# leggedrobotics/wild_visual_navigation

Measured on NVIDIA H100. Metric: frames/sec end-to-end (DINO feat + seg + MLP train-step) at 448x448, higher is better.
Workload: dtype bf16 operands / fp32 accumulate (ViT, STEGO head, per-pixel MLP); fp32 (k-means, train step)

## Files before the change

wild_visual_navigation_b200/csrc/attention_wgmma.cu:

```cuda
#include <stdlib.h>

#include "attention.h"
#include "common.cuh"
#include "host_common.h"

namespace wvn {

namespace {

constexpr int kThreads = 384;
constexpr int kConsumerWarps = 8;
constexpr int kTileQ = 128;
constexpr int kTileKV = 128;
constexpr int kDh = 64;
constexpr uint32_t kQBytes = kTileQ * kDh * 2;
constexpr uint32_t kKBytes = kTileKV * kDh * 2;
constexpr uint32_t kVBytes = kDh * kTileKV * 2;
constexpr int kStages = 4;
constexpr uint32_t kOffQ = 0;
constexpr uint32_t kOffK = kOffQ + kQBytes;
constexpr uint32_t kOffV = kOffK + kStages * kKBytes;
constexpr uint32_t kOffBar = kOffV + kStages * kVBytes;
constexpr uint32_t kSmemBytes = kOffBar + 256 + 1024 ;

__device__ __forceinline__ float fast_exp2(float x) {
  float y;
  asm("ex2.approx.ftz.f32 %0, %1;" : "=f"(y) : "f"(x));
  return y;
}

__device__ __forceinline__ float quad_max(float v) {
  v = fmaxf(v, __shfl_xor_sync(0xffffffffu, v, 1));
  return fmaxf(v, __shfl_xor_sync(0xffffffffu, v, 2));
}

template <bool MASKED>
__device__ __forceinline__ void softmax_scores(float (&s)[64], float (&m)[2], float (&l)[2], float (&alpha)[2],
                                               const float sl2, const int valid, const int q) {
  if (MASKED) {
#pragma unroll
    for (int j = 0; j < 16; ++j)
#pragma unroll
      for (int e = 0; e < 2; ++e)
        if (8 * j + 2 * q + e >= valid) s[4 * j + e] = s[4 * j + 2 + e] = -INFINITY;
  }
  float neg_m[2];
#pragma unroll
  for (int h = 0; h < 2; ++h) {
    float mx = s[2 * h];
#pragma unroll
    for (int j = 0; j < 16; ++j) mx = fmaxf(mx, fmaxf(s[4 * j + 2 * h], s[4 * j + 2 * h + 1]));
    mx = fmaxf(quad_max(mx), m[h]);
    alpha[h] = fast_exp2((m[h] - mx) * sl2);
    m[h] = mx;
    neg_m[h] = -mx * sl2;
  }
  float sum[2] = {0.f, 0.f};
#pragma unroll
  for (int j = 0; j < 16; ++j) {
#pragma unroll
    for (int h = 0; h < 2; ++h) {
      const float e0 = fast_exp2(fmaf(s[4 * j + 2 * h], sl2, neg_m[h]));
      const float e1 = fast_exp2(fmaf(s[4 * j + 2 * h + 1], sl2, neg_m[h]));
      sum[h] += e0 + e1;
      s[4 * j + 2 * h] = e0;
      s[4 * j + 2 * h + 1] = e1;
    }
  }
#pragma unroll
  for (int h = 0; h < 2; ++h) l[h] = fmaf(l[h], alpha[h], sum[h]);
}

__device__ __forceinline__ void rescale_o(float (&o)[32], const float (&alpha)[2]) {
#pragma unroll
  for (int j = 0; j < 8; ++j) {
    o[4 * j + 0] *= alpha[0];
    o[4 * j + 1] *= alpha[0];
    o[4 * j + 2] *= alpha[1];
    o[4 * j + 3] *= alpha[1];
  }
}

__device__ __forceinline__ void pack_p(const float (&s)[64], uint32_t (&p)[32]) {
#pragma unroll
  for (int j = 0; j < 16; ++j)
#pragma unroll
    for (int h = 0; h < 2; ++h)
      p[4 * (j >> 1) + 2 * (j & 1) + h] = pack_bf16x2(s[4 * j + 2 * h], s[4 * j + 2 * h + 1]);
}

__global__ void __launch_bounds__(kThreads, 1)
attention_kernel(const __grid_constant__ CUtensorMap tmap_q, const __grid_constant__ CUtensorMap tmap_k,
                 const __grid_constant__ CUtensorMap tmap_v, const AttnArgs args) {
  extern __shared__ uint8_t smem_raw[];
  uint8_t* smem = reinterpret_cast<uint8_t*>((reinterpret_cast<uintptr_t>(smem_raw) + 1023) & ~uintptr_t(1023));
  uint64_t* bars = reinterpret_cast<uint64_t*>(smem + kOffBar);
  uint64_t* q_full = bars;
  uint64_t* kv_full = bars + 1;
  uint64_t* kv_empty = bars + 1 + kStages;

  const int warp = threadIdx.x >> 5, lane = threadIdx.x & 31;
  const int ntiles = args.npad / kTileQ;
  const int q_tile = args.reverse ? ntiles - 1 - static_cast<int>(blockIdx.x) : static_cast<int>(blockIdx.x);
  const int bh = args.reverse ? static_cast<int>(gridDim.y) - 1 - static_cast<int>(blockIdx.y) : static_cast<int>(blockIdx.y);
  const int num_kv = args.npad / kTileKV;

  if (threadIdx.x == 0) {
    tma_prefetch_desc(&tmap_q);
    tma_prefetch_desc(&tmap_k);
    tma_prefetch_desc(&tmap_v);
    mbar_init(q_full, 1);
    for (int i = 0; i < kStages; ++i) {
      mbar_init(&kv_full[i], 1);
      mbar_init(&kv_empty[i], kConsumerWarps);
    }
    fence_mbar_init();
  }
  __syncthreads();

  if (warp < 4) {
    setmaxnreg_dec<40>();
    if (warp == 0) {
      if (elect_one_sync()) {
        mbar_arrive_expect_tx(q_full, kQBytes);
        tma_load_2d(&tmap_q, q_full, smem + kOffQ, 0, bh * args.npad + q_tile * kTileQ);
      }
      __syncwarp();
      int stage = 0;
      uint32_t phase = 0;
      for (int j = 0; j < num_kv; ++j) {
        mbar_wait(&kv_empty[stage], phase ^ 1);
        if (elect_one_sync()) {
          mbar_arrive_expect_tx(&kv_full[stage], kKBytes + kVBytes);
          tma_load_2d(&tmap_k, &kv_full[stage], smem + kOffK + stage * kKBytes, 0, bh * args.npad + j * kTileKV);
          tma_load_2d(&tmap_v, &kv_full[stage], smem + kOffV + stage * kVBytes, j * kTileKV, bh * kDh);
          tma_load_2d(&tmap_v, &kv_full[stage], smem + kOffV + stage * kVBytes + kVBytes / 2, j * kTileKV + 64, bh * kDh);
        }
        __syncwarp();
        if (++stage == kStages) { stage = 0; phase ^= 1; }
      }
    }
  } else {
    setmaxnreg_inc<232>();
    const int cwarp = warp - 4;
    const int wg = cwarp >> 2;
    const int q = lane & 3;
    const float sl2 = args.scale_log2;
    float s[64], o[32];
    uint32_t p[32];
    float m[2] = {-INFINITY, -INFINITY}, l[2] = {0.f, 0.f};

    float alpha[2];

    mbar_wait(q_full, 0);
    const uint64_t desc_q = make_sw128_kmajor_desc(smem_u32(smem + kOffQ + wg * 64 * 128));
    auto issue_qk = [&](int st) {
      const uint64_t desc_k = make_sw128_kmajor_desc(smem_u32(smem + kOffK + st * kKBytes));
#pragma unroll
      for (int k = 0; k < kDh / 16; ++k) wgmma_m64n128k16_ss(s, desc_q + 2 * k, desc_k + 2 * k, k != 0 ? 1u : 0u);
      wgmma_commit();
    };
    auto issue_pv = [&](int st, bool accumulate) {
      const uint32_t v_addr = smem_u32(smem + kOffV + st * kVBytes);
#pragma unroll
      for (int k = 0; k < kTileKV / 16; ++k)
        wgmma_m64n64k16_rs(o, p[4 * k], p[4 * k + 1], p[4 * k + 2], p[4 * k + 3],
                           make_sw128_kmajor_desc(v_addr + (k >> 2) * (kVBytes / 2)) + 2 * (k & 3),
                           (accumulate || k != 0) ? 1u : 0u);
      wgmma_commit();
    };
    auto take_turn = [&]() { named_bar_sync(1 + wg, 256); };
    auto pass_turn = [&](bool last) { if (!(last && wg == 1)) named_bar_arrive(2 - wg, 256); };
    if (wg == 1) named_bar_arrive(1, 256);

    mbar_wait(&kv_full[0], 0);
    take_turn();
    wgmma_fence_regs(s);
    wgmma_fence();
    issue_qk(0);
    pass_turn(false);
    wgmma_wait<0>();
    wgmma_fence_regs(s);
    if (num_kv == 1) softmax_scores<true>(s, m, l, alpha, sl2, args.n_valid, q);
    else softmax_scores<false>(s, m, l, alpha, sl2, kTileKV, q);
    pack_p(s, p);

    int stage = 0;
    uint32_t phase = 0;
    for (int j = 1; j < num_kv; ++j) {
      const int prev_stage = stage;
      if (++stage == kStages) { stage = 0; phase ^= 1; }
      mbar_wait(&kv_full[stage], phase);
      take_turn();
      wgmma_fence_regs(s);
      wgmma_fence_regs(o);
      wgmma_fence();
      issue_qk(stage);
      issue_pv(prev_stage, j > 1);
      pass_turn(false);
      wgmma_wait<1>();
      wgmma_fence_regs(s);
      if (j == num_kv - 1) softmax_scores<true>(s, m, l, alpha, sl2, args.n_valid - j * kTileKV, q);
      else softmax_scores<false>(s, m, l, alpha, sl2, kTileKV, q);
      wgmma_wait<0>();
      wgmma_fence_regs(o);
      wgmma_fence_regs(p);
      if (lane == 0) mbar_arrive(&kv_empty[prev_stage]);
      rescale_o(o, alpha);
      pack_p(s, p);
    }
    take_turn();
    wgmma_fence_regs(o);
    wgmma_fence();
    issue_pv(stage, num_kv > 1);
    pass_turn(true);
    wgmma_wait<0>();
    wgmma_fence_regs(o);

    const int frame = bh / args.heads, head = bh - frame * args.heads;
    const int row0 = q_tile * kTileQ + wg * 64 + (cwarp & 3) * 16 + (lane >> 2);
#pragma unroll
    for (int h = 0; h < 2; ++h) {
      float lt = l[h];
      lt += __shfl_xor_sync(0xffffffffu, lt, 1);
      lt += __shfl_xor_sync(0xffffffffu, lt, 2);
      const float inv = 1.f / lt;
      __nv_bfloat16* dst = reinterpret_cast<__nv_bfloat16*>(args.out) +
                           (static_cast<long long>(frame) * args.npad + row0 + 8 * h) * args.ldo + head * kDh + 2 * q;
#pragma unroll
      for (int jj = 0; jj < 8; ++jj)
        *reinterpret_cast<uint32_t*>(dst + 8 * jj) = pack_bf16x2(o[4 * jj + 2 * h] * inv, o[4 * jj + 2 * h + 1] * inv);
    }
  }
}

}

int attention_bf16(const AttnArgs& a, const void* q, const void* k, const void* vt, cudaStream_t stream) {
  WVN_REQUIRE(a.batch > 0 && a.heads > 0, "attention: empty problem");
  WVN_REQUIRE(a.npad % kTileKV == 0 && a.n_valid > 0 && a.n_valid <= a.npad && a.n_valid > a.npad - kTileKV,
              "attention: npad=%d must be a multiple of 128 and n_valid=%d must lie in the last tile", a.npad,
              a.n_valid);
  const long long bh = static_cast<long long>(a.batch) * a.heads;
  WVN_REQUIRE(bh <= 65535, "attention: batch * heads = %lld exceeds the grid's y extent", bh);
  CUtensorMap tq, tk, tv;
  WVN_PROPAGATE(make_tmap_bf16_2d(&tq, q, kDh, bh * a.npad, kDh * 2, 64, kTileQ));
  WVN_PROPAGATE(make_tmap_bf16_2d(&tk, k, kDh, bh * a.npad, kDh * 2, 64, kTileKV));
  WVN_PROPAGATE(make_tmap_bf16_2d(&tv, vt, a.npad, bh * kDh, static_cast<uint64_t>(a.npad) * 2, 64, kDh));
  static bool attr_set = false;
  if (!attr_set) {
    WVN_CHECK_CUDA(cudaFuncSetAttribute(attention_kernel, cudaFuncAttributeMaxDynamicSharedMemorySize, kSmemBytes));
    attr_set = true;
  }
  dim3 grid(a.npad / kTileQ, static_cast<unsigned>(bh));
  prof_begin(PROF_ATTENTION, stream);
  attention_kernel<<<grid, kThreads, kSmemBytes, stream>>>(tq, tk, tv, a);
  prof_end(PROF_ATTENTION, stream);
  WVN_CHECK_LAUNCH("attention_kernel");
  return WVN_OK;
}

}
```

Before: 974.6.

## Make attention kernel persistent with double-buffered Q and TMA output stores

Converts the attention kernel to a persistent grid sized to the SM count. Each CTA loops over (batch*head, q-tile) units, with a double-buffered Q tile so the next unit's first QK^T overlaps the previous unit's final PV. Output is staged through swizzled shared memory and written with TMA stores instead of direct global stores. This aims to remove launch/tail and prologue/epilogue bubbles per tile, at the cost of more shared memory and more complex barrier phase tracking.

```diff
diff --git a/wild_visual_navigation_b200/csrc/attention_wgmma.cu b/wild_visual_navigation_b200/csrc/attention_wgmma.cu
--- a/wild_visual_navigation_b200/csrc/attention_wgmma.cu
+++ b/wild_visual_navigation_b200/csrc/attention_wgmma.cu
@@ -1,4 +1,7 @@
+#include <stdint.h>
 #include <stdlib.h>
+
+#include <algorithm>
 
 #include "attention.h"
 #include "common.cuh"
@@ -16,11 +19,14 @@
 constexpr uint32_t kQBytes = kTileQ * kDh * 2;
 constexpr uint32_t kKBytes = kTileKV * kDh * 2;
 constexpr uint32_t kVBytes = kDh * kTileKV * 2;
+constexpr uint32_t kOBytes = kTileQ * kDh * 2;
+constexpr int kQBufs = 2;
 constexpr int kStages = 4;
 constexpr uint32_t kOffQ = 0;
-constexpr uint32_t kOffK = kOffQ + kQBytes;
+constexpr uint32_t kOffK = kOffQ + kQBufs * kQBytes;
 constexpr uint32_t kOffV = kOffK + kStages * kKBytes;
-constexpr uint32_t kOffBar = kOffV + kStages * kVBytes;
+constexpr uint32_t kOffO = kOffV + kStages * kVBytes;
+constexpr uint32_t kOffBar = kOffO + kOBytes;
 constexpr uint32_t kSmemBytes = kOffBar + 256 + 1024 ;
 
 __device__ __forceinline__ float fast_exp2(float x) {
@@ -91,25 +97,35 @@
 
 __global__ void __launch_bounds__(kThreads, 1)
 attention_kernel(const __grid_constant__ CUtensorMap tmap_q, const __grid_constant__ CUtensorMap tmap_k,
-                 const __grid_constant__ CUtensorMap tmap_v, const AttnArgs args) {
+                 const __grid_constant__ CUtensorMap tmap_v, const __grid_constant__ CUtensorMap tmap_o,
+                 const AttnArgs args) {
   extern __shared__ uint8_t smem_raw[];
   uint8_t* smem = reinterpret_cast<uint8_t*>((reinterpret_cast<uintptr_t>(smem_raw) + 1023) & ~uintptr_t(1023));
   uint64_t* bars = reinterpret_cast<uint64_t*>(smem + kOffBar);
   uint64_t* q_full = bars;
-  uint64_t* kv_full = bars + 1;
-  uint64_t* kv_empty = bars + 1 + kStages;
+  uint64_t* q_empty = bars + kQBufs;
+  uint64_t* kv_full = bars + 2 * kQBufs;
+  uint64_t* kv_empty = bars + 2 * kQBufs + kStages;
 
   const int warp = threadIdx.x >> 5, lane = threadIdx.x & 31;
   const int ntiles = args.npad / kTileQ;
-  const int q_tile = args.reverse ? ntiles - 1 - static_cast<int>(blockIdx.x) : static_cast<int>(blockIdx.x);
-  const int bh = args.reverse ? static_cast<int>(gridDim.y) - 1 - static_cast<int>(blockIdx.y) : static_cast<int>(blockIdx.y);
   const int num_kv = args.npad / kTileKV;
+  const int units = args.batch * args.heads * ntiles;
+  auto unit_coords = [&](int u, int& bh, int& q_tile) {
+    const int ue = args.reverse ? units - 1 - u : u;
+    bh = ue / ntiles;
+    q_tile = ue - bh * ntiles;
+  };
 
   if (threadIdx.x == 0) {
     tma_prefetch_desc(&tmap_q);
     tma_prefetch_desc(&tmap_k);
     tma_prefetch_desc(&tmap_v);
-    mbar_init(q_full, 1);
+    tma_prefetch_desc(&tmap_o);
+    for (int i = 0; i < kQBufs; ++i) {
+      mbar_init(&q_full[i], 1);
+      mbar_init(&q_empty[i], kConsumerWarps);
+    }
     for (int i = 0; i < kStages; ++i) {
       mbar_init(&kv_full[i], 1);
       mbar_init(&kv_empty[i], kConsumerWarps);
@@ -121,23 +137,31 @@
   if (warp < 4) {
     setmaxnreg_dec<40>();
     if (warp == 0) {
-      if (elect_one_sync()) {
-        mbar_arrive_expect_tx(q_full, kQBytes);
-        tma_load_2d(&tmap_q, q_full, smem + kOffQ, 0, bh * args.npad + q_tile * kTileQ);
-      }
-      __syncwarp();
       int stage = 0;
       uint32_t phase = 0;
-      for (int j = 0; j < num_kv; ++j) {
-        mbar_wait(&kv_empty[stage], phase ^ 1);
+      int it = 0;
+      for (int u = blockIdx.x; u < units; u += gridDim.x, ++it) {
+        int bh, q_tile;
+        unit_coords(u, bh, q_tile);
+        const int qb = it & 1;
+        mbar_wait(&q_empty[qb], ((it >> 1) & 1) ^ 1);
         if (elect_one_sync()) {
-          mbar_arrive_expect_tx(&kv_full[stage], kKBytes + kVBytes);
-          tma_load_2d(&tmap_k, &kv_full[stage], smem + kOffK + stage * kKBytes, 0, bh * args.npad + j * kTileKV);
-          tma_load_2d(&tmap_v, &kv_full[stage], smem + kOffV + stage * kVBytes, j * kTileKV, bh * kDh);
-          tma_load_2d(&tmap_v, &kv_full[stage], smem + kOffV + stage * kVBytes + kVBytes / 2, j * kTileKV + 64, bh * kDh);
+          mbar_arrive_expect_tx(&q_full[qb], kQBytes);
+          tma_load_2d(&tmap_q, &q_full[qb], smem + kOffQ + qb * kQBytes, 0, bh * args.npad + q_tile * kTileQ);
         }
         __syncwarp();
-        if (++stage == kStages) { stage = 0; phase ^= 1; }
+        for (int j = 0; j < num_kv; ++j) {
+          mbar_wait(&kv_empty[stage], phase ^ 1);
+          if (elect_one_sync()) {
+            mbar_arrive_expect_tx(&kv_full[stage], kKBytes + kVBytes);
+            tma_load_2d(&tmap_k, &kv_full[stage], smem + kOffK + stage * kKBytes, 0, bh * args.npad + j * kTileKV);
+            tma_load_2d(&tmap_v, &kv_full[stage], smem + kOffV + stage * kVBytes, j * kTileKV, bh * kDh);
+            tma_load_2d(&tmap_v, &kv_full[stage], smem + kOffV + stage * kVBytes + kVBytes / 2, j * kTileKV + 64,
+                        bh * kDh);
+          }
+          __syncwarp();
+          if (++stage == kStages) { stage = 0; phase ^= 1; }
+        }
       }
     }
   } else {
@@ -145,16 +169,12 @@
     const int cwarp = warp - 4;
     const int wg = cwarp >> 2;
     const int q = lane & 3;
+    const bool leader = (threadIdx.x & 127) == 0;
     const float sl2 = args.scale_log2;
     float s[64], o[32];
     uint32_t p[32];
-    float m[2] = {-INFINITY, -INFINITY}, l[2] = {0.f, 0.f};
-
-    float alpha[2];
-
-    mbar_wait(q_full, 0);
-    const uint64_t desc_q = make_sw128_kmajor_desc(smem_u32(smem + kOffQ + wg * 64 * 128));
-    auto issue_qk = [&](int st) {
+
+    auto issue_qk = [&](uint64_t desc_q, int st) {
       const uint64_t desc_k = make_sw128_kmajor_desc(smem_u32(smem + kOffK + st * kKBytes));
 #pragma unroll
       for (int k = 0; k < kDh / 16; ++k) wgmma_m64n128k16_ss(s, desc_q + 2 * k, desc_k + 2 * k, k != 0 ? 1u : 0u);
@@ -172,65 +192,123 @@
     auto take_turn = [&]() { named_bar_sync(1 + wg, 256); };
     auto pass_turn = [&](bool last) { if (!(last && wg == 1)) named_bar_arrive(2 - wg, 256); };
     if (wg == 1) named_bar_arrive(1, 256);
-
-    mbar_wait(&kv_full[0], 0);
+    auto q_desc = [&](int it) {
+      return make_sw128_kmajor_desc(smem_u32(smem + kOffQ + (it & 1) * kQBytes + wg * 64 * 128));
+    };
+    float m[2], l[2], alpha[2];
+    auto first_softmax = [&]() {
+      m[0] = m[1] = -INFINITY;
+      l[0] = l[1] = 0.f;
+      if (num_kv == 1) softmax_scores<true>(s, m, l, alpha, sl2, args.n_valid, q);
+      else softmax_scores<false>(s, m, l, alpha, sl2, kTileKV, q);
+    };
+
+    int stage = 0;
+    uint32_t phase = 0;
+    int it = 0;
+    int u = blockIdx.x;
+    mbar_wait(&q_full[0], 0);
+    mbar_wait(&kv_full[stage], phase);
     take_turn();
     wgmma_fence_regs(s);
     wgmma_fence();
-    issue_qk(0);
+    issue_qk(q_desc(0), stage);
     pass_turn(false);
     wgmma_wait<0>();
     wgmma_fence_regs(s);
-    if (num_kv == 1) softmax_scores<true>(s, m, l, alpha, sl2, args.n_valid, q);
-    else softmax_scores<false>(s, m, l, alpha, sl2, kTileKV, q);
+    first_softmax();
     pack_p(s, p);
 
-    int stage = 0;
-    uint32_t phase = 0;
-    for (int j = 1; j < num_kv; ++j) {
-      const int prev_stage = stage;
+    for (;;) {
+      const uint64_t desc_q = q_desc(it);
+      for (int j = 1; j < num_kv; ++j) {
+        const int prev_stage = stage;
+        if (++stage == kStages) { stage = 0; phase ^= 1; }
+        mbar_wait(&kv_full[stage], phase);
+        take_turn();
+        wgmma_fence_regs(s);
+        wgmma_fence_regs(o);
+        wgmma_fence();
+        issue_qk(desc_q, stage);
+        issue_pv(prev_stage, j > 1);
+        pass_turn(false);
+        wgmma_wait<1>();
+        wgmma_fence_regs(s);
+        if (j == num_kv - 1) softmax_scores<true>(s, m, l, alpha, sl2, args.n_valid - j * kTileKV, q);
+        else softmax_scores<false>(s, m, l, alpha, sl2, kTileKV, q);
+        wgmma_wait<0>();
+        wgmma_fence_regs(o);
+        wgmma_fence_regs(p);
+        if (lane == 0) mbar_arrive(&kv_empty[prev_stage]);
+        rescale_o(o, alpha);
+        pack_p(s, p);
+      }
+      if (lane == 0) mbar_arrive(&q_empty[it & 1]);
+
+      const int next = u + static_cast<int>(gridDim.x);
+      const bool has_next = next < units;
+      const int last_stage = stage;
       if (++stage == kStages) { stage = 0; phase ^= 1; }
-      mbar_wait(&kv_full[stage], phase);
-      take_turn();
-      wgmma_fence_regs(s);
-      wgmma_fence_regs(o);
-      wgmma_fence();
-      issue_qk(stage);
-      issue_pv(prev_stage, j > 1);
-      pass_turn(false);
-      wgmma_wait<1>();
-      wgmma_fence_regs(s);
-      if (j == num_kv - 1) softmax_scores<true>(s, m, l, alpha, sl2, args.n_valid - j * kTileKV, q);
-      else softmax_scores<false>(s, m, l, alpha, sl2, kTileKV, q);
-      wgmma_wait<0>();
-      wgmma_fence_regs(o);
-      wgmma_fence_regs(p);
-      if (lane == 0) mbar_arrive(&kv_empty[prev_stage]);
-      rescale_o(o, alpha);
-      pack_p(s, p);
-    }
-    take_turn();
-    wgmma_fence_regs(o);
-    wgmma_fence();
-    issue_pv(stage, num_kv > 1);
-    pass_turn(true);
-    wgmma_wait<0>();
-    wgmma_fence_regs(o);
-
-    const int frame = bh / args.heads, head = bh - frame * args.heads;
-    const int row0 = q_tile * kTileQ + wg * 64 + (cwarp & 3) * 16 + (lane >> 2);
-#pragma unroll
-    for (int h = 0; h < 2; ++h) {
-      float lt = l[h];
-      lt += __shfl_xor_sync(0xffffffffu, lt, 1);
-      lt += __shfl_xor_sync(0xffffffffu, lt, 2);
-      const float inv = 1.f / lt;
-      __nv_bfloat16* dst = reinterpret_cast<__nv_bfloat16*>(args.out) +
-                           (static_cast<long long>(frame) * args.npad + row0 + 8 * h) * args.ldo + head * kDh + 2 * q;
-#pragma unroll
-      for (int jj = 0; jj < 8; ++jj)
-        *reinterpret_cast<uint32_t*>(dst + 8 * jj) = pack_bf16x2(o[4 * jj + 2 * h] * inv, o[4 * jj + 2 * h + 1] * inv);
-    }
+      const float l_unit[2] = {l[0], l[1]};
+      if (has_next) {
+        mbar_wait(&q_full[(it + 1) & 1], ((it + 1) >> 1) & 1);
+        mbar_wait(&kv_full[stage], phase);
+        take_turn();
+        wgmma_fence_regs(s);
+        wgmma_fence_regs(o);
+        wgmma_fence();
+        issue_qk(q_desc(it + 1), stage);
+        issue_pv(last_stage, num_kv > 1);
+        pass_turn(false);
+        wgmma_wait<1>();
+        wgmma_fence_regs(s);
+        first_softmax();
+        wgmma_wait<0>();
+        wgmma_fence_regs(o);
+        wgmma_fence_regs(p);
+        if (lane == 0) mbar_arrive(&kv_empty[last_stage]);
+        pack_p(s, p);
+      } else {
+        take_turn();
+        wgmma_fence_regs(o);
+        wgmma_fence();
+        issue_pv(last_stage, num_kv > 1);
+        pass_turn(true);
+        wgmma_wait<0>();
+        wgmma_fence_regs(o);
+        if (lane == 0) mbar_arrive(&kv_empty[last_stage]);
+      }
+
+      int bh, q_tile;
+      unit_coords(u, bh, q_tile);
+      const int frame = bh / args.heads, head = bh - frame * args.heads;
+      const uint32_t staging = smem_u32(smem + kOffO) + wg * (kOBytes / 2);
+      const int r0 = (cwarp & 3) * 16 + (lane >> 2);
+      if (leader) tma_store_wait_read<0>();
+      named_bar_sync(3 + wg, 128);
+#pragma unroll
+      for (int h = 0; h < 2; ++h) {
+        float lt = l_unit[h];
+        lt += __shfl_xor_sync(0xffffffffu, lt, 1);
+        lt += __shfl_xor_sync(0xffffffffu, lt, 2);
+        const float inv = 1.f / lt;
+        const int r = r0 + 8 * h;
+#pragma unroll
+        for (int jj = 0; jj < 8; ++jj)
+          sts32(staging + r * 128 + ((jj ^ (r & 7)) << 4) + 4 * q,
+                pack_bf16x2(o[4 * jj + 2 * h] * inv, o[4 * jj + 2 * h + 1] * inv));
+      }
+      fence_proxy_async_smem();
+      named_bar_sync(3 + wg, 128);
+      if (leader) {
+        tma_store_2d(&tmap_o, staging, head * kDh, frame * args.npad + q_tile * kTileQ + wg * 64);
+        tma_store_commit();
+      }
+      if (!has_next) break;
+      u = next;
+      ++it;
+    }
+    if (leader) tma_store_wait_all<0>();
   }
 }
 
@@ -242,19 +320,22 @@
               "attention: npad=%d must be a multiple of 128 and n_valid=%d must lie in the last tile", a.npad,
               a.n_valid);
   const long long bh = static_cast<long long>(a.batch) * a.heads;
-  WVN_REQUIRE(bh <= 65535, "attention: batch * heads = %lld exceeds the grid's y extent", bh);
-  CUtensorMap tq, tk, tv;
+  const long long units = bh * (a.npad / kTileQ);
+  WVN_REQUIRE(bh * a.npad <= INT32_MAX && units <= INT32_MAX, "attention: batch * heads = %lld is too large", bh);
+  CUtensorMap tq, tk, tv, to;
   WVN_PROPAGATE(make_tmap_bf16_2d(&tq, q, kDh, bh * a.npad, kDh * 2, 64, kTileQ));
   WVN_PROPAGATE(make_tmap_bf16_2d(&tk, k, kDh, bh * a.npad, kDh * 2, 64, kTileKV));
   WVN_PROPAGATE(make_tmap_bf16_2d(&tv, vt, a.npad, bh * kDh, static_cast<uint64_t>(a.npad) * 2, 64, kDh));
+  WVN_PROPAGATE(make_tmap_bf16_2d(&to, a.out, static_cast<uint64_t>(a.heads) * kDh,
+                                  static_cast<uint64_t>(a.batch) * a.npad, static_cast<uint64_t>(a.ldo) * 2, 64, 64));
   static bool attr_set = false;
   if (!attr_set) {
     WVN_CHECK_CUDA(cudaFuncSetAttribute(attention_kernel, cudaFuncAttributeMaxDynamicSharedMemorySize, kSmemBytes));
     attr_set = true;
   }
-  dim3 grid(a.npad / kTileQ, static_cast<unsigned>(bh));
+  const int grid = static_cast<int>(std::min<long long>(sm_count(), units));
   prof_begin(PROF_ATTENTION, stream);
-  attention_kernel<<<grid, kThreads, kSmemBytes, stream>>>(tq, tk, tv, a);
+  attention_kernel<<<grid, kThreads, kSmemBytes, stream>>>(tq, tk, tv, to, a);
   prof_end(PROF_ATTENTION, stream);
   WVN_CHECK_LAUNCH("attention_kernel");
   return WVN_OK;
```

Measured after the change: 985.8 (median of 6 runs). About the same (+1.1%).
